# QuakeMigrate/QuakeMigrate

Measured on AMD Instinct MI355X. Metric: grid-nodes x time-samples stacked /sec (detect sweep), higher is better.
Workload: dtype f64

## Files before the change

quakemigrate_amd/csrc/qm_config.hip:

```cpp
#include "qm_config.hpp"

#include <cstring>

namespace {

using C = EngineConfig;

constexpr Tunable flag(const char *name, int C::*m, unsigned effects = 0) {
    return {name, m, nullptr, Tunable::kFlag, 0, 1, 0, {}, nullptr, effects};
}
constexpr Tunable range(const char *name, int C::*m, int64_t lo, int64_t hi, const char *refusal, unsigned effects = 0) {
    return {name, m, nullptr, Tunable::kRange, lo, hi, 0, {}, refusal, effects};
}
constexpr Tunable one_of(const char *name, int C::*m, int a, int b, int c, int d, const char *refusal,
                         unsigned effects = 0) {
    return {name, m, nullptr, Tunable::kSet, a, d, 4, {a, b, c, d}, refusal, effects};
}

}

const Tunable kTunables[] = {
    range("brick_x", &C::brick_x, 0, 64, "brick_x must be in 0..64 (0 = automatic)"),
    range("brick_y", &C::brick_y, 0, 64, "brick_y must be in 0..64 (0 = automatic)"),
    range("brick_z", &C::brick_z, 0, 64, "brick_z must be in 0..64 (0 = automatic)"),
    one_of("samples_per_lane", &C::samples_per_lane, 0, 1, 2, 4, "samples_per_lane must be 0 (automatic), 1, 2 or 4"),
    range("waves", &C::waves, 1, 16, "waves must be 1..16", kUserWaves),
    {"groups", &C::groups, nullptr, Tunable::kAtLeast, 0, 0, 0, {}, "groups must be >= 0", 0},
    range("rounds", &C::rounds, 1, 1024, "rounds must be in 1..1024", kUserRounds),
    range("lds_bytes", &C::lds_bytes, 1024, 160 * 1024, "lds_bytes must be in 1 KiB..160 KiB", kUserLds),
    flag("force_direct", &C::force_direct),
    flag("generic", &C::generic),
    flag("exact", &C::exact),
    range("scan_waves", &C::scan_waves, 1, 4096, "scan_waves must be in 1..4096"),
    {"chunk_bytes", nullptr, &C::chunk_bytes, Tunable::kAtLeast, 1 << 20, 0, 0, {}, "chunk_bytes must be >= 1 MiB", 0},
    range("pair", &C::pair, 0, 2, "pair must be 0 (off), 1 (automatic) or 2 (any scan length)"),
    flag("screen", &C::screen),
    one_of("screen_pairs", &C::screen_pairs, 0, 1, 2, 4, "screen_pairs must be 0, 1, 2 or 4", kVoidScreen),
    flag("screen_brick16", &C::screen_brick16, kVoidScreen),
    range("screen_big", &C::screen_big, -1, 1, "screen_big must be -1 (automatic), 0 or 1", kVoidScreen),
    range("shift", &C::shift, -1, 1, "shift must be -1 (automatic), 0 (off) or 1"),
    one_of("shift_waves", &C::shift_waves, 0, 4, 8, 12, "shift_waves must be 0 (automatic), 4, 8 or 12", kVoidShift),
    range("shift_lazy", &C::shift_lazy, -1, 1, "shift_lazy must be -1 (automatic), 0 or 1"),
    flag("shift_tail", &C::shift_tail),
    range("shift_rows_direct", &C::shift_rows_direct, 0, 2, "shift_rows_direct must be 0, 1 or 2", kVoidShift),
    range("shift_wide", &C::shift_wide, -1, 1, "shift_wide must be -1 (automatic), 0 (off) or 1"),
    range("shift_wide_rows", &C::shift_wide_rows, 0, 2,
          "shift_wide_rows must be 0 (never), 1 (where all rows do not fit) or 2 (always)", kVoidShiftWide),
    range("stream_pull", &C::stream_pull, -1, 1, "stream_pull must be -1 (slots of <= 1 MB), 0 (never) or 1 (always)"),
    flag("stream_stamps", &C::stream_stamps),
    flag("preproc_skew", &C::preproc_skew),
    range("tie_rule", &C::tie_rule, 0, 1, "tie_rule must be 0 (largest sum) or 1 (the reference's exp rule)"),
    flag("tie_sets", &C::tie_sets),
    flag("trigger_timing", &C::trigger_timing),
    flag("log_timing", &C::log_timing, kResetTimingLog),
};
const int kNumTunables = (int)(sizeof(kTunables) / sizeof(kTunables[0]));

static const Tunable *find_tunable(const char *key) {
    for (const Tunable &t : kTunables)
        if (std::strcmp(t.name, key) == 0) return &t;
    return nullptr;
}

int config_set(EngineConfig &c, const char *key, int64_t v, unsigned *effects) {
    const Tunable *t = find_tunable(key);
    if (!t) return fail("unknown config key '%s'", key);
    bool ok = true;
    switch (t->check) {
    case Tunable::kFlag: v = v ? 1 : 0; break;
    case Tunable::kRange: ok = v >= t->lo && v <= t->hi; break;
    case Tunable::kAtLeast: ok = v >= t->lo; break;
    case Tunable::kSet:
        ok = false;
        for (int i = 0; i < t->n_allowed; ++i) ok = ok || v == t->allowed[i];
        break;
    }
    if (!ok) return fail("%s", t->refusal);
    if (t->wide) c.*t->wide = v;
    else c.*t->member = (int)v;
    if (t->member == &C::lds_bytes) c.lds_bytes = (int)(v / 16 * 16);
    if ((t->member == &C::brick_x || t->member == &C::brick_y || t->member == &C::brick_z) && c.brick_x > 0) {
        if (c.brick_y < 1) c.brick_y = 1;
        if (c.brick_z < 1) c.brick_z = 1;
    }
    if (t->effects & kUserWaves) c.user_waves = true;
    if (t->effects & kUserRounds) c.user_rounds = true;
    if (t->effects & kUserLds) c.user_lds = true;
    if (effects) *effects = t->effects;
    return 0;
}

bool config_get(const EngineConfig &c, const char *key, int64_t *v) {
    const Tunable *t = find_tunable(key);
    if (!t) return false;
    *v = t->wide ? c.*t->wide : (int64_t)(c.*t->member);
    return true;
}
```

quakemigrate_amd/csrc/qm_config.hpp:

```cpp
#pragma once
#include <cstdint>

#pragma GCC visibility push(hidden)

int fail(const char *fmt, ...) __attribute__((format(printf, 1, 2)));

struct EngineConfig {
    int brick_x = 0, brick_y = 0, brick_z = 0;
    int samples_per_lane = 0;
    int waves = 8;
    bool user_waves = false, user_lds = false;
    int groups = 0;
    int rounds = 12;
    bool user_rounds = false;
    int lds_bytes = 80 * 1024;
    int force_direct = 0;
    int generic = 0;
    int scan_waves = 32;
    int exact = 1;
    int64_t chunk_bytes = (int64_t)4 << 30;
    int pair = 1;
    int screen = 0;
    int screen_pairs = 0;
    int screen_brick16 = 0;
    int screen_big = -1;
    int shift = -1;
    int shift_waves = 0;
    int shift_lazy = -1;
    int shift_tail = 1;
    int shift_rows_direct = 1;
    int shift_wide = -1;
    int shift_wide_rows = 1;
    int stream_pull = -1;
    int stream_stamps = 0;
    int preproc_skew = 1;
    int tie_rule = 0;
    int tie_sets = 1;
    int trigger_timing = 0;
    int log_timing = 0;
};

enum ConfigEffect : unsigned {
    kVoidShift = 1u << 0,
    kVoidShiftWide = 1u << 1,
    kVoidScreen = 1u << 2,
    kUserWaves = 1u << 3,
    kUserRounds = 1u << 4,
    kUserLds = 1u << 5,
    kResetTimingLog = 1u << 6,
};

struct Tunable {
    enum Check { kFlag, kRange, kAtLeast, kSet };
    const char *name;
    int EngineConfig::*member;
    int64_t EngineConfig::*wide;
    Check check;
    int64_t lo, hi;
    int n_allowed;
    int allowed[4];
    const char *refusal;
    unsigned effects;
};
extern const Tunable kTunables[];
extern const int kNumTunables;

int config_set(EngineConfig &c, const char *key, int64_t v, unsigned *effects);
bool config_get(const EngineConfig &c, const char *key, int64_t *v);

#pragma GCC visibility pop
```

quakemigrate_amd/csrc/qm_engine.hip:

```cpp
#define QM_TU_STEPS 1
#include "qm_engine.hpp"

namespace {

using qm::kPairLdsBytes;

qm::LaunchShape stack_shape(const qm_engine *e, const qm::StackArgs &a, int threads, size_t lds) {
    const int steps = a.n_steps > 1 ? a.n_steps : 1;
    return {(unsigned)(steps * a.ntiles * ((a.ngroups + 7) / 8 * 8)), threads, lds, e->stream};
}

bool pair_built(int S) { return S >= 1 && S <= qm::kPairMaxRows; }


bool shift_wanted(const qm_engine *e, int n_chunk, bool plain, bool volume, int64_t vol_stride) {
    if (!plain || e->cfg.shift == 0 || e->cfg.generic || e->cfg.force_direct ||
        e->cfg.user_waves || e->cfg.user_lds || e->cfg.samples_per_lane > 0 || e->cfg.pair == 2)
        return false;
    if (volume && vol_stride * 8 >= ((int64_t)1 << 32)) return false;
    if ((int64_t)e->g.ny * e->g.nz * 8 >= ((int64_t)1 << 32)) return false;
    return n_chunk >= 1;
}

int shift_tail_spl(const qm_engine *e, int rest) {
// ... 88 lines not shown
        p.cap_doubles = kPairLdsBytes / 8;
    }
    if (s.n_steps > 1) {
        p.batched = !volume && !marginal && !accumulate && s.run_if == nullptr && want_scan && (!shift || L->plain());
        if (!p.batched) {
            *out = p;
            return 0;
        }
        p.steps = s.n_steps;
    }
    if (!shift && jp == 0) {
        if (J != 1 && J != 2 && J != 4) return fail("samples_per_lane must be 1, 2 or 4 (got %d)", J);
        if (ensure_rel(e)) return 1;
    }
    if (marginal) p.marg_tiles = p.ntiles;
    const int n_wide_now = p.layout->n_list, nbricks_now = p.layout->g.nbricks;
    p.use_direct = e->cfg.force_direct || n_wide_now > 0;
    p.use_lds = !e->cfg.force_direct && n_wide_now < nbricks_now;
    p.direct_j = shift ? 4 : jp > 0 ? 2 * jp : J;
    p.direct_threads = shift ? 512 : jp > 0 ? 1024 : run_waves(e) * qm::kWave;
    p.direct_publish = (size_t)3 * (p.direct_threads / qm::kWave) * qm::kWave * p.direct_j * sizeof(double);
    const int threads = p.direct_threads;
    const int lds_blocks_per_cu =
        shift ? (L->nw == qm::kShiftWaves ? 2 : 1) : jp > 0 ? 1
               : std::max(1, std::min(160 * 1024 / std::max(1, run_lds_bytes(e)), 2048 / threads));
    if (p.use_lds) {
        int rounds = (!shift && jp == 0 && !e->cfg.user_rounds && e->g.brick_nodes <= 64) ? 3 : 0;
        if (shift && (wide || (L->nw == qm::kShiftWaves8 && L->nblk == 1)) && !e->cfg.user_rounds) {
            double best = 1e300;
            for (int r = 1; r <= e->cfg.rounds; ++r) {
                const int g = auto_groups(e, p.ntiles, nbricks_now, lds_blocks_per_cu, r);
                const double busy = (double)p.ntiles * g / ((double)r * e->n_cu * lds_blocks_per_cu);
                const double cost = (1.0 - std::min(1.0, busy)) + 0.002 * r;
                if (cost < best - 1e-9) { best = cost; rounds = r; }
            }
        }
        p.groups_lds = e->cfg.groups > 0 ? std::min(e->cfg.groups, nbricks_now)
                                         : auto_groups(e, p.ntiles, nbricks_now, lds_blocks_per_cu, rounds);
        p.brick_rows = (e->cfg.tie_rule && want_scan && e->cfg.tie_sets && shift && p.shift_mode == qm::kShiftDetect &&
                        L->plain()) ? nbricks_now : 0;
        if (e->cfg.tie_rule && want_scan && !p.brick_rows && !e->cfg.user_rounds && e->cfg.groups == 0) {
            const int fine = auto_groups(e, p.ntiles, std::max(1, nbricks_now / 4), lds_blocks_per_cu,
                                         8 * (rounds > 0 ? rounds : e->cfg.rounds));
            p.groups_lds = std::max(p.groups_lds, fine);
        }
        if (shift) {
            p.family = kFamilyShift;
            p.j = p.wide_tiles > 0 ? qm::kShiftWideSpl : 4;
            const bool per_brick = p.brick_rows && p.wide_tiles == 0;
            const int64_t life = (per_brick ? 1 : (int64_t)L->g.nbricks / std::max(1, p.groups_lds)) *
                                 std::max(1, L->g.brick_nodes / 8 / L->nw);
            p.lazy = e->cfg.shift_lazy >= 0 ? e->cfg.shift_lazy : (life >= qm::kShiftLazyGroups ? 1 : 0);
            if (L->nblk > 1 && !L->direct) p.lazy = 0;
        } else if (jp > 0) {
            p.family = kFamilyPair;
            p.j = 2 * jp;
        } else {
            const int S = e->g.n_rows;
            const bool exact = e->cfg.exact && !e->cfg.generic && !accumulate && qm::exact_built(S, J) &&
                               (marginal || !volume || S > qm::kPairMaxRows);
            p.family = exact ? kFamilyExact : kFamilyChunked;
            p.j = J;
        }
    }
    if (p.use_direct) {
        const int units = e->cfg.force_direct ? nbricks_now : n_wide_now;
        p.groups_direct = e->cfg.groups > 0 ? std::min(e->cfg.groups, units)
                                            : auto_groups(e, p.ntiles, units, 2048 / threads);
        p.list = e->cfg.force_direct ? nullptr : p.layout->list.p;
        p.n_list = units;
    }
    p.g = p.layout->g;
    p.sets = p.groups_lds + p.groups_direct;
    p.scan_n = p.steps * n_chunk;
    *out = p;
    return 0;
}

qm::StackArgs stack_args(const qm_engine *e, const StackLaunch &s, const StackPlan &p, bool direct) {
    const auto *vol = std::get_if<StackLaunch::Volume>(&s.kind);
    const auto *marg = std::get_if<StackLaunch::Marginal>(&s.kind);
    qm::StackArgs a{};
    a.g = p.g;
    a.onsets = s.onsets;
    a.lut = e->d_lut.p;
    if (!p.shift) {
        a.rel = p.layout->rel.p;
        a.brick_meta = p.layout->meta.p;
        a.brick_total = p.layout->total.p;
    }
    a.brick_list = direct ? p.list : nullptr;
    a.n_list = direct ? p.n_list : 0;
    a.T = s.T;
    a.fsmp = s.fsmp;
    a.n_samples = s.n_samples;
    a.sample0 = s.sample0;
    a.n_chunk = s.n_chunk;
    a.ntiles = direct && p.shift ? (s.n_chunk + qm::kShiftKT - 1) / qm::kShiftKT : p.ntiles;
    a.ngroups = direct ? p.groups_direct : p.groups_lds;
    a.tail_spl = direct ? 0 : p.tail_spl;
    a.wide_tiles = direct ? 0 : p.wide_tiles;
    if (p.steps > 1) {
        a.n_steps = p.steps;
        a.step_stride = s.step_stride;
    }
    a.part_stride = p.scan_n;
    a.cap_doubles = p.cap_doubles;
    a.z_scale = 1.4426950408889634074 / (double)s.available;
    a.volume = vol ? vol->p : nullptr;
    a.vol_stride = vol ? vol->stride : 0;
    a.accumulate = vol ? vol->accumulate : 0;
    a.part_max = e->d_pmax.p;
    a.part_idx = e->d_pidx.p;
    a.part_sum = e->d_psum.p;
    a.set0 = direct && p.use_lds ? p.groups_lds : 0;
    a.brick_max = p.brick_rows && !direct ? e->d_bmax.p : nullptr;
    a.want_scan = s.want_scan ? 1 : 0;
    a.marginal = marg ? e->d_marg.p : nullptr;
    a.m0 = marg ? marg->first : 0;
    a.m1 = marg ? marg->end : 0;
    a.n_nodes = e->n_nodes;
    a.run_if = s.run_if;
    return a;
}

int launch_round2_lds(qm_engine *e, const qm::StackArgs &a, StackPlan *p) {
    const int J = p->j, S = e->g.n_rows;
    const bool VOLUME = a.volume != nullptr || a.marginal != nullptr;
    const qm::LaunchShape shape = stack_shape(e, a, p->direct_threads,
                                              std::max((size_t)run_lds_bytes(e), p->direct_publish));
    bool exact = false;
    if (p->family == kFamilyExact) {
        const bool j4_wide = J == 4 && S > 40;
        if (a.marginal != nullptr) {
            if (S <= 32) QM_TABLE(qm::launch_exact_marginal_1_32(S, a, shape, &exact));
            else if (!j4_wide) QM_TABLE(qm::launch_exact_marginal_33_64(S, a, shape, &exact));
            else QM_TABLE(qm::launch_exact_marginal_j4_41_64(S, a, shape, &exact));
        } else if (!VOLUME) {
            if (S <= 32) QM_TABLE(qm::launch_exact_detect_1_32(S, a, shape, &exact));
            else if (!j4_wide) QM_TABLE(qm::launch_exact_detect_33_64(S, a, shape, &exact));
            else QM_TABLE(qm::launch_exact_detect_j4_41_64(S, a, shape, &exact));
        } else {
            if (!j4_wide) QM_TABLE(qm::launch_exact_volume_33_64(S, a, shape, &exact));
            else QM_TABLE(qm::launch_exact_volume_j4_41_64(S, a, shape, &exact));
        }
    }
    if (!exact) {
        p->family = kFamilyChunked;
        int nch = (e->cfg.generic || a.accumulate) ? 0 : e->g.row_pad / 8;
        if (nch > 8) nch = 0;
        bool built = false;
        if (VOLUME) QM_TABLE(qm::launch_chunked_volume(J, nch, a, shape, &built));
        else QM_TABLE(qm::launch_chunked_detect(J, nch, a, shape, &built));
        if (!built) return fail("no chunked stacking kernel for %d samples per lane", J);
    }
    return 0;
}

int launch_pair_lds(qm_engine *e, const qm::StackArgs &a) {
    bool done = false;
    const qm::LaunchShape shape = stack_shape(e, a, 1024, kPairLdsBytes);
    if (a.volume) QM_TABLE(qm::launch_pair_volume(e->g.n_rows, a, shape, &done));
    else QM_TABLE(qm::launch_pair_detect(e->g.n_rows, a, shape, &done));
    if (!done) return fail("no paired kernel built for %d rows", e->g.n_rows);
    return 0;
}

int launch_shift_lds(qm_engine *e, const qm::StackArgs &a, const StackPlan &p) {
    const ShiftLayout &L = *p.shift;
    const int mode = p.shift_mode;
    qm::ShiftArgs s{};
    s.a = a;
    s.smeta = reinterpret_cast<const int4 *>(L.meta.p);
    s.stotal = L.total.p;
    s.sfit = L.fit.p;
    s.stream = reinterpret_cast<const char *>(L.stream.p);
    s.wmeta = reinterpret_cast<const int4 *>(L.wmeta.p);
    s.wtotal = L.wtotal.p;
    s.wstream = reinterpret_cast<const char *>(L.wstream.p);
    s.rows2 = L.rows2;
    s.nw = L.nw;
    s.nblk = L.nblk;
    s.sb = L.sb;
    s.stage_slots = L.stage_slots;
    s.stage_reach = L.stage_reach;
    s.lazy = p.lazy;
    const qm::LaunchShape shape = stack_shape(e, a, L.nw * qm::kWave, qm::shift_lds_bytes(L.nw));
    const bool rows = L.nblk > 1, big = L.nw == qm::kShiftWaves8;
    if (L.wide && L.direct) QM_TABLE(qm::launch_shift_wide_rows(s, shape));
    else if (rows && L.quad && mode == qm::kShiftVolume) QM_TABLE(qm::launch_shift_rows4_volume(s, shape));
    else if (rows && L.quad) QM_TABLE(qm::launch_shift_rows4(s, shape));
    else if (rows && L.direct && mode == qm::kShiftVolume) QM_TABLE(qm::launch_shift_rows2_volume(s, shape));
    else if (rows && L.direct) QM_TABLE(qm::launch_shift_rows2(s, shape));
    else if (rows) QM_TABLE(qm::launch_shift_rows8(s, shape));
    else if (mode == qm::kShiftMarginal && big) QM_TABLE(qm::launch_shift_marginal8(s, shape));
    else if (mode == qm::kShiftMarginal) QM_TABLE(qm::launch_shift_marginal(s, shape));
    else if (mode == qm::kShiftVolume && big) QM_TABLE(qm::launch_shift_volume8(s, shape));
    else if (mode == qm::kShiftVolume) QM_TABLE(qm::launch_shift_volume(s, shape));
    else if (L.nw == qm::kShiftWaves3) QM_TABLE(qm::launch_shift_detect3(s, shape));
    else if (a.brick_max && big) QM_TABLE(qm::launch_shift_detect8_sets(s, shape));
    else if (a.brick_max) QM_TABLE(qm::launch_shift_detect_sets(s, shape));
    else if (big) QM_TABLE(qm::launch_shift_detect8(s, shape));
    else QM_TABLE(qm::launch_shift_detect(s, shape));
    return 0;
}

int launch_direct(qm_engine *e, const qm::StackArgs &a, const StackPlan &p) {
    const qm::LaunchShape shape = stack_shape(e, a, p.direct_threads, p.direct_publish);
    bool built = false;
    if (a.volume || a.marginal) QM_TABLE(qm::launch_direct_volume(p.direct_j, a, shape, &built));
    else QM_TABLE(qm::launch_direct_detect(p.direct_j, a, shape, &built));
    if (!built) return fail("no direct stacking kernel for %d samples per lane", p.direct_j);
    return 0;
}

int issue_stack(qm_engine *e, const StackLaunch &s, StackPlan *p) {
    if (p->marg_tiles && e->d_marg.ensure((size_t)p->marg_tiles * e->n_nodes)) return 1;
    const size_t rows_n = (size_t)p->brick_rows * p->scan_n;
    if (s.want_scan) {
        const size_t need = (size_t)p->sets * p->scan_n;
        if (e->d_pmax.ensure(need) || e->d_psum.ensure(need) || e->d_pidx.ensure(need)) return 1;
        if (p->brick_rows && e->d_bmax.ensure(rows_n)) return 1;
    }
    if (p->brick_rows && p->wide_tiles > 0) {
        hipLaunchKernelGGL(qm::fill_kernel, dim3((unsigned)std::min<size_t>((rows_n + 1023) / 1024, 65535)), dim3(256),
                           0, e->stream, e->d_bmax.p, rows_n, -std::numeric_limits<double>::infinity());
        QM_HIP(hipGetLastError());
    }
    const bool logged = s.run_if == nullptr;
    hipEvent_t ev_begin = nullptr, ev_end = nullptr;
    if (logged) {
        if (timing_events(e, &ev_begin, &ev_end)) return 1;
        QM_HIP(hipEventRecord(ev_begin, e->stream));
    }
    if (p->use_lds) {
        const qm::StackArgs a = stack_args(e, s, *p, false);
        if (p->family == kFamilyShift ? launch_shift_lds(e, a, *p)
            : p->family == kFamilyPair ? launch_pair_lds(e, a) : launch_round2_lds(e, a, p))
            return 1;
    }
    if (p->use_direct && launch_direct(e, stack_args(e, s, *p, true), *p)) return 1;
    if (logged) {
        QM_HIP(hipEventRecord(ev_end, e->stream));
        e->timed = !e->cfg.log_timing;
    }
    return 0;
}

}

int timing_events(qm_engine *e, hipEvent_t *begin, hipEvent_t *end) {
    *begin = e->ev0;
    *end = e->ev1;
    if (!e->cfg.log_timing) return 0;
    while (e->ev_used + 2 > e->ev_log.size()) {
        Event ev;
        QM_HIP(ev.create());
        e->ev_log.push_back(std::move(ev));
    }
    *begin = e->ev_log[e->ev_used];
    *end = e->ev_log[e->ev_used + 1];
    e->ev_used += 2;
    return 0;
}

StackResult run_stack(qm_engine *e, const StackLaunch &s) {
    e->last.sets_own = false;
    StackPlan p;
    if (plan_stack(e, s, &p)) return 1;
    StackResult r;
    r.batched = p.batched;
    if (!p.batched) return r;
    if (issue_stack(e, s, &p)) return 1;
    e->last = p;
    r.sets = p.sets;
    return r;
}

SetView engine_sets(const qm_engine *e, int n_sets, int n) {
// ... 172 lines not shown
}

int fetch_out(qm_engine *e, int n, int out_on_device, const OutSeries &st, const OutSeries &user) {
    if (out_on_device) return 0;
    void *dst[3] = {user.max, user.second, user.idx};
    QM_HIP(copy_back_pieces(dst, st.max, 3, (size_t)n * sizeof(double), e->stream));
    return 0;
}

namespace {

int finalize_sets(qm_engine *e, const SetView &in, int64_t n_nodes_total, const OutSeries &user, int out_on_device) {
    DeviceGuard guard(e->device);
    OutSeries st;
    if (stage_out(e, in.n, out_on_device, user, &st) || combine(e, in, kCombineFinal, 0, n_nodes_total, st, nullptr))
        return 1;
    return fetch_out(e, in.n, out_on_device, st, user);
}

struct Readout {
    const char *name;
    int64_t (*value)(const qm_engine *e);
    int (*fetch)(qm_engine *e);
};
int fetch_tie_counts(qm_engine *e) {
    if (!e->tie.counts_pending) return 0;
    int32_t h[2] = {0, 0};
    QM_HIP(copy_back(h, e->tie.count.p, sizeof(h), e->stream));
    e->tie.pairs_last = h[0];
    e->tie.overflow_last = h[1];
    e->tie.counts_pending = false;
    return 0;
}
#define V(expr) [](const qm_engine *e) -> int64_t { return (expr); }
const Readout kReadouts[] = {
    {"waves", V(run_waves(e))}, {"lds_bytes", V(run_lds_bytes(e))},
    {"screen_pairs", V(e->sweep.last_plan_jp)}, {"screen_big", V(e->sweep.last_plan_big)},
    {"shift_waves", V(e->last.shift && e->last.shift->ok ? e->last.shift->nw : e->sh.ok ? e->sh.nw : e->cfg.shift_waves)},
    {"screened_steps", V(e->sweep.screened_steps), drain_flags}, {"fallback_steps", V(e->sweep.fallback_steps), drain_flags},
    {"last_candidates", V(e->sweep.last_candidates), drain_flags}, {"screen_brick_nodes", V(e->screen.g.brick_nodes)},
    {"last_kernel", V(e->last.family)}, {"last_kernel_j", V(e->last.j)}, {"steps_per_launch", V(e->last_batched)},
    {"shift_tail_spl", V(e->last.tail_spl)}, {"shift_wide_tiles", V(e->last.wide_tiles)},
    {"shift_ok", V(e->sh.built && e->sh.ok ? 1 : 0)}, {"shift_wide_ok", V(e->shw.built && e->shw.ok ? 1 : 0)},
    {"shift_row_blocks", V(e->sh.ok ? e->sh.nblk : 0)}, {"shift_wide_row_blocks", V(e->shw.ok ? e->shw.nblk : 0)},
    {"shift_brick_nodes", V(e->sh.ok ? e->sh.g.brick_nodes : 0)},
    {"shift_wide_brick_nodes", V(e->shw.ok ? e->shw.g.brick_nodes : 0)},
    {"shift_wide_bricks", V(e->sh.ok ? e->sh.n_list : 0)}, {"shift_wide_direct_bricks", V(e->shw.ok ? e->shw.n_list : 0)},
    {"shift_operands_per_add_x1000",
     V(e->sh.ok && e->sh.group_rows > 0 ? (e->sh.quads * 4 * 1000) / (e->sh.group_rows * 32) : 0)},
    {"shift_wide_operands_per_add_x1000",
     V(e->shw.ok && e->shw.group_rows > 0 ? (e->shw.wquads * 4 * 1000) / (e->shw.group_rows * 48) : 0)},
    {"pair_brick_nodes", V(e->pair.kt ? e->pair.g.brick_nodes : 0)}, {"pair_tile", V(e->pair.ok ? e->pair.kt : 0)},
    {"pair_wide_bricks", V(e->pair.kt ? e->pair.n_list : 0)}, {"shift_lazy", V(e->last.lazy)},
    {"pick_lds_samples", V(qm::kPicksLdsSamples)}, {"amp_lds_samples", V(qm::kAmpLdsSamples)},
    {"trigger_max_radius", V(qm::kTrigMaxRadius)}, {"trigger_smooth_tile", V(qm::kTrigSmoothTile)},
    {"trigger_run_block", V(qm::kTrigRunBlock)}, {"trigger_merge_stride", V(qm::kTrigMergeThreads)},
    {"scanmseed_tile", V(qm::kSmsTile)}, {"scanmseed_compose_chunk", V(qm::kSmsComposeChunk)},
    {"tt_lds_nodes", V(qm::kTtLdsNodes)}, {"tt_section_threads", V(qm::kTtSectionThreads)},
    {"tt_grid_blocks", V(qm::kTtGridBlocks)}, {"tt_grid_threads", V(qm::kTtGridThreads)},
    {"tie_brick_rows", V(e->last.brick_rows)}, {"tie_refined_steps", V(e->tie.refined_steps)},
    {"tie_overflow_samples", V(e->tie.overflow_last), fetch_tie_counts}, {"tie_pairs", V(e->tie.pairs_last), fetch_tie_counts},
    {"table_hits", V(e->table_hits)}, {"table_misses", V(e->table_misses)}, {"table_evictions", V(e->table_evictions)},
    {"table_digests", V(e->table_digests)}, {"table_bytes", V(e->device_bytes())},
    {"tables_parked", V(std::count_if(e->slots.begin(), e->slots.end(), [](const TableSlot &sl) { return sl.used; }))},
    {"tables_parked_bytes", [](const qm_engine *e) -> int64_t {
         int64_t sum = 0;
         for (const TableSlot &sl : e->slots) sum += sl.used ? (int64_t)sl.state.device_bytes() : 0;
         return sum;
     }},
    {"pool_live_bytes", V(pool_live_bytes(e->device))},
    {"n_bricks", V(e->g.nbricks)},
    {"n_wide_bricks", V(e->r2().n_list), [](qm_engine *e) { return e->have_lut ? plan_wide(e, eff_j(e)) : 0; }},
    {"mean_span", [](const qm_engine *e) -> int64_t {
         int64_t sum = 0;
         const std::vector<int32_t> &totals = e->r2().h_total;
         for (int32_t t : totals) sum += t;
         return totals.empty() ? 0 : sum / ((int64_t)totals.size() * std::max(1, e->g.n_rows));
     }},
    {"n_cu", V(e->n_cu)}, {"n_nodes", V(e->n_nodes)}, {"n_rows", V(e->g.n_rows)},
    {"nx", V(e->g.nx)}, {"ny", V(e->g.ny)}, {"nz", V(e->g.nz)},
};
#undef V

template <int N>
bool clock_readout(const StageClock<N> &clock, const std::string &prefix, const std::string &key, int64_t *v) {
    for (int st = 0; st < N; ++st)
        if (key == prefix + clock.names[st]) return *v = clock.ns[st], true;
    return false;
}

}

extern "C" {

int qm_engine_create(int device_id, qm_engine **out) {
    if (!out) return fail("qm_engine_create: out is NULL");
    int n = 0;
    QM_HIP(hipGetDeviceCount(&n));
    if (device_id < 0 || device_id >= n)
        return fail("device %d not available (%d HIP devices visible)", device_id, n);
    DeviceGuard guard(device_id);
    std::unique_ptr<qm_engine, decltype(&qm_engine_destroy)> e(new qm_engine(), qm_engine_destroy);
    e->device = device_id;
    hipDeviceProp_t prop;
    QM_HIP(hipGetDeviceProperties(&prop, device_id));
    e->n_cu = prop.multiProcessorCount > 0 ? prop.multiProcessorCount : 256;
// ... 349 lines not shown
```

quakemigrate_amd/csrc/qm_engine.hpp:

```cpp
#pragma once
#include "../../include/qmhip.h"

#include <hip/hip_runtime.h>

#include <algorithm>
#include <atomic>
#include <cmath>
#include <cstdarg>
#include <cstdio>
#include <cstdlib>
#include <cstring>
#include <memory>
#include <mutex>
#include <string>
#include <thread>
#include <variant>
#include <vector>

#include "qm_config.hpp"
#include "qm_kernels.hpp"
#include "qm_launch.hpp"
#include "qm_screen.hpp"
#include "qm_pair.hpp"
#include "qm_shift.hpp"
// ... 310 lines not shown
    DevBuf<double> par;
    DevBuf<double> sec, out;
    DevBuf<double> tau;
    DevBuf<int32_t> meta;
    DevBuf<unsigned long long> bad;
    StageClock<qm::kTtStages> clock{qm::kTtStageNames};
};
struct TieScratch {
    DevBuf<double> zext, zgrid, z;
    DevBuf<int32_t> pairs, imin, count, cands;
    DevBuf<unsigned long long> emax, keys;
    int64_t refined_steps = 0, overflow_last = 0, pairs_last = 0;
    bool counts_pending = false;
};
struct ScreenScratch {
    DevBuf<int32_t> counts, cells, work, flags;
    DevBuf<int32_t> onq, cell, gmax, pm, sparams;
    DevBuf<double> rowmax, ssum, cand_z;
    DevBuf<int64_t> cand_idx;
    int64_t screened_steps = 0, fallback_steps = 0, last_candidates = 0;
    int last_plan_jp = 0, last_plan_big = 0;
    PinnedBuf<int32_t> h_flags;
    int flags_pending = 0, flags_head = 0;
};
struct FitScratch {
    DevBuf<double> a, b, c;
    DevBuf<double> part, val, win;
    DevBuf<int64_t> pidx;
};
struct CallStaging {
    DevBuf<double> sig;
    DevBuf<double> raw;
    DevBuf<double> pre_out;
    DevBuf<double> rs_raw;
};

struct StreamLane;

enum StackFamily : int { kFamilyChunked = 0, kFamilyExact = 1, kFamilyPair = 2, kFamilyShift = 3 };
struct StackPlan {
    StackFamily family = kFamilyChunked;
    int j = 0;
    const BrickLayout *layout = nullptr;
    const ShiftLayout *shift = nullptr;
    int shift_mode = 0, lazy = 0;
    int tail_spl = 0, wide_tiles = 0;
    int ntiles = 0, cap_doubles = 0;
    int steps = 1;
    bool use_lds = false, use_direct = false;
    int groups_lds = 0, groups_direct = 0;
    int direct_j = 0, direct_threads = 0;
    size_t direct_publish = 0;
    int brick_rows = 0;
    int marg_tiles = 0;
    bool batched = true;
    qm::GridDesc g{};
    const int32_t *list = nullptr;
    int n_list = 0;
    int sets = 0, scan_n = 0;
    bool sets_own = false;
};

struct qm_engine : TableState {
    int device = 0;
    std::vector<StreamLane *> streams;
    int n_cu = 256;
    hipStream_t own_stream = nullptr;
    hipStream_t stream = nullptr;
    Event ev0, ev1;
    bool timed = false;
    std::vector<Event> ev_log;
    size_t ev_used = 0;

    std::vector<TableSlot> slots;
    uint64_t cur_key = 0, table_clock = 0;
    bool cur_keyed = false;
    int64_t table_hits = 0, table_misses = 0, table_evictions = 0;
    int64_t table_digests = 0;
    DevBuf<unsigned long long> d_digest;

    EngineConfig cfg;

    DevBuf<int32_t> d_scalar;
    int last_batched = 1;
    StackPlan last;

    DevBuf<double> d_grids;
    DevBuf<int32_t> d_rows, d_served;
    int gx = 0, gy = 0, gz = 0, g_rows = 0;

    DevBuf<double> d_onsets, d_pmax, d_psum, d_bmax, d_out_a, d_chunk, d_marg, d_marg_out;
    DevBuf<int64_t> d_pidx;

    ResampleStage rs_stage;
    PreprocStage pre_stage;
    OnsetStage on_stage;
    CallStaging staging;
    PickStage picks;
    AmplitudeStage amps;
    TriggerStage trig;
    ScanmseedCodec sms;
    TravelTimeStage tt;
    TieScratch tie;
    ScreenScratch sweep;
    FitScratch fit;
};
// ... 188 lines not shown
```

quakemigrate_amd/csrc/qm_kernels.hpp:

```cpp
#pragma once

#include <hip/hip_runtime.h>
#include <stdint.h>

namespace qm {

constexpr int kWave = 64;
constexpr int64_t kNoIndex = INT64_MAX;
constexpr int kMaxSpanBytes = 65535;

struct GridDesc {
    int nx, ny, nz;
    int bx, by, bz;
    int nbx, nby, nbz;
    int nbricks;
    int brick_nodes;
    int n_rows;
    int row_pad;
};

struct StackArgs {
    GridDesc g;
    const double *onsets;
    const int32_t *lut;
    const uint16_t *rel;
    const int32_t *brick_meta;
    const int32_t *brick_total;
    const int32_t *brick_list;
    int n_list;
    int T, fsmp, n_samples;
    int sample0;
    int n_chunk;
    int ntiles, ngroups;
    int tail_spl;
    int wide_tiles;
    int n_steps;
    int64_t step_stride;
    int64_t part_stride;
    int cap_doubles;
    double z_scale;
    double *volume;
    int64_t vol_stride;
    int accumulate;
    double *part_max;
    int64_t *part_idx;
    double *part_sum;
    int set0;
    double *brick_max;
    int want_scan;
    double *marginal;
    int m0, m1;
    int64_t n_nodes;
    const int32_t *run_if;
};

__device__ __forceinline__ double max_keep(double best, double x) {
    double r;
    asm("v_max_f64 %0, %1, %2" : "=v"(r) : "v"(best), "v"(x));
    return r;
}

template <typename I>
__device__ __forceinline__ bool better(double v, I i, double best, I bi) {
    return (v > best) || (v == best && i < bi);
}

__device__ __forceinline__ void stack_tile_group(const StackArgs &a, int &tile, int &group) {
    const int slot = blockIdx.x >> 3;
    const int all = a.ntiles * (a.n_steps > 1 ? a.n_steps : 1);
    tile = (slot % all) % a.ntiles;
    group = (int)(blockIdx.x & 7) + 8 * (slot / all);
}
__device__ __forceinline__ StackArgs step_view(StackArgs a) {
    if (a.part_stride == 0) a.part_stride = a.n_chunk;
    if (a.n_steps > 1) {
        const int step = (int)((blockIdx.x >> 3) % (unsigned)(a.ntiles * a.n_steps)) / a.ntiles;
        a.onsets += (int64_t)step * a.step_stride;
        a.part_max += (int64_t)step * a.n_chunk;
        a.part_idx += (int64_t)step * a.n_chunk;
        a.part_sum += (int64_t)step * a.n_chunk;
        if (a.brick_max) a.brick_max += (int64_t)step * a.n_chunk;
    }
    return a;
}

__host__ __device__ __forceinline__ bool brick_fits(int64_t total_span, int n_rows, int kt,
                                                    int cap_doubles) {
    return total_span * 8 <= kMaxSpanBytes && total_span + (int64_t)n_rows * kt <= cap_doubles;
}

__device__ __forceinline__ void brick_extents(const GridDesc &g, int b, int &x0, int &y0, int &z0,
                                              int &vx, int &vy, int &vz) {
    const int bzi = b % g.nbz, byi = (b / g.nbz) % g.nby, bxi = b / (g.nbz * g.nby);
    x0 = bxi * g.bx; y0 = byi * g.by; z0 = bzi * g.bz;
    vx = min(g.bx, g.nx - x0); vy = min(g.by, g.ny - y0); vz = min(g.bz, g.nz - z0);
}

__device__ __forceinline__ int brick_walk_node(const GridDesc &g, int x0, int y0, int z0, int vy,
                                               int vz, int m) {
    const int lz = m % vz, ly = (m / vz) % vy, lx = m / (vz * vy);
    return ((x0 + lx) * g.ny + (y0 + ly)) * g.nz + (z0 + lz);
}

#ifdef QM_TU_TABLES
__global__ void brick_minmax_kernel(GridDesc g, const int32_t *__restrict__ lut,
                                    int4 *__restrict__ meta, int32_t *__restrict__ global_max) {
    const int b = blockIdx.x;
    int x0, y0, z0, vx, vy, vz;
    brick_extents(g, b, x0, y0, z0, vx, vy, vz);
    const int nvalid = vx * vy * vz;
    for (int r = threadIdx.x; r < g.n_rows; r += blockDim.x) {
        int lo = INT32_MAX, hi = 0;
        for (int m = 0; m < nvalid; ++m) {
            const int node = brick_walk_node(g, x0, y0, z0, vy, vz, m);
            int d = lut[(int64_t)node * g.n_rows + r];
            d = d < 0 ? 0 : d;
            lo = d < lo ? d : lo;
            hi = d > hi ? d : hi;
        }
        meta[(int64_t)b * g.n_rows + r] = make_int4(lo, hi - lo, 0, 0);
        atomicMax(global_max, hi);
    }
}
#endif

#ifdef QM_TU_TABLES
__global__ void brick_prefix_kernel(GridDesc g, int4 *__restrict__ meta,
                                    int32_t *__restrict__ btotal) {
    const int b = blockIdx.x * blockDim.x + threadIdx.x;
    if (b >= g.nbricks) return;
    int64_t run = 0;
    for (int r = 0; r < g.n_rows; ++r) {
        meta[(int64_t)b * g.n_rows + r].z = (int32_t)(run > INT32_MAX ? INT32_MAX : run);
        run += meta[(int64_t)b * g.n_rows + r].y;
// ... 1220 lines not shown
```

quakemigrate_amd/csrc/qm_shift.hpp:

```cpp
#pragma once

#include "qm_kernels.hpp"

namespace qm {

struct ShiftStageNext {
    const void *meta;
    int rows;
    int first_row, stride;
    const void *src;
    unsigned row_bytes;
    unsigned lds;
    unsigned lane32;
};

#ifndef QM_SHIFT_ASM_INC
#define QM_SHIFT_ASM_INC "qm_shift_asm.inc"
#endif
#include QM_SHIFT_ASM_INC

constexpr int kShiftWaves = 4;
constexpr int kShiftWaves8 = 8;
constexpr int kShiftWaves3 = 12;
constexpr int kShiftKT = 256;
// ... 329 lines not shown
                             "s_mov_b32 m0, %[ma]\n\t"
                             "s_nop 0\n\t"
                             "global_load_lds_dwordx4 %[vo], %[src]\n\t"
                             "s_mov_b64 exec, %[sv]"
                             : [sv] "=&s"(saved)
                             : [sh] "s"(__builtin_amdgcn_readfirstlane(kWave - pairs)),
                               [ma] "s"(__builtin_amdgcn_readfirstlane((int)(lds_base + 8u * (unsigned)(z4 + c)))),
                               [vo] "v"(lane16), [src] "s"(usrc + c)
                             : "memory", "m0");
            }
        } else {
            const int len = __builtin_amdgcn_readfirstlane(m.y) + kShiftWideKT;
            for (int u = lane; u < total; u += kWave) win[z4 + u] = (u < len && u < room) ? src[u] : 0.0;
        }
    }
    if ((S & 1) && wave == 0) {
        const int z4 = 4 * s.wtotal[vb];
        for (int u = lane; u < 4 * shift_zero_slots(1); u += kWave) win[z4 + u] = 0.0;
    }
}

struct ShiftWork {
    int tile, group, spl;
    int t_own;
    int t_first;
    bool run;
};
__device__ __forceinline__ ShiftWork shift_work(const StackArgs &a) {
    ShiftWork w;
    stack_tile_group(a, w.tile, w.group);
    w.run = w.group < a.ngroups && !(a.run_if != nullptr && *a.run_if == 0);
    if (w.tile < a.wide_tiles) {
        w.spl = kShiftWideSpl;
        w.t_own = w.tile * kShiftWideKT;
        w.t_first = w.t_own + kShiftWideKT > a.n_chunk ? a.n_chunk - kShiftWideKT : w.t_own;
        return w;
    }
    w.spl = (a.tail_spl > 0 && w.tile == a.ntiles - 1) ? a.tail_spl : 4;
    w.t_own = a.wide_tiles * kShiftWideKT + (w.tile - a.wide_tiles) * kShiftKT;
    w.t_first = (w.spl == 4 && w.t_own + kShiftKT > a.n_chunk && a.n_chunk >= kShiftKT)
                    ? a.n_chunk - kShiftKT : w.t_own;
    return w;
}
template <int J>
__device__ __forceinline__ void shift_reset(double (&vmax)[J], double (&vsum)[J], int (&vidx)[J]) {
#pragma unroll
    for (int k = 0; k < J; ++k) {
        vmax[k] = -__builtin_inf();
        vsum[k] = 0.0;
        vidx[k] = INT32_MAX;
    }
}

template <int NW, int J = 4>
__device__ __forceinline__ void shift_publish(const StackArgs &a, double *win, const double (&vmax)[J],
                                              const double (&vsum)[J], const int (&vidx)[J], int wave,
                                              int lane, int group, int t_first, int t_own = 0) {
    constexpr int KT = kWave * J;
    double *smax = win, *ssum = win + NW * KT;
    int *sidx = reinterpret_cast<int *>(win + 2 * NW * KT);
#pragma unroll
    for (int k = 0; k < J; ++k) {
        const int o = wave * KT + J * lane + k;
        smax[o] = vmax[k];
        ssum[o] = vsum[k];
        sidx[o] = vidx[k];
    }
    __syncthreads();
    const int k = threadIdx.x;
    if (k >= KT) return;
    double best = smax[k], total = ssum[k];
    int bi = sidx[k];
    for (int w = 1; w < NW; ++w) {
        const double v = smax[w * KT + k];
        const int i = sidx[w * KT + k];
        total += ssum[w * KT + k];
        if (better(v, i, best, bi)) {
            best = v;
            bi = i;
        }
    }
    const int t = t_first + k;
    if (t < a.n_chunk && t >= t_own) {
        const int64_t o = (int64_t)(a.set0 + group) * (a.part_stride ? a.part_stride : a.n_chunk) + t;
        a.part_max[o] = best;
        a.part_idx[o] = bi == INT32_MAX ? kNoIndex : (int64_t)bi;
        a.part_sum[o] = total;
    }
}

template <int MODE, int NW, int J, bool WIDE_LAZY = false, int SETS = 0>
__device__ __forceinline__ void shift_tile(const ShiftArgs &s, double *win, const ShiftWork &work,
                                           int lane, int wave) {
    constexpr bool kLdsState = NW == kShiftWaves3;
    constexpr bool kWide = J == kShiftWideSpl;
    constexpr bool kTail = J != 4;
    static_assert(!(kTail && kLdsState), "the 12-wave shape has no tail flavours");
    static_assert(!kWide || (MODE == kShiftDetect && NW == kShiftWaves8), "wide tiles: fused detect, 8 waves");
    static_assert(!SETS || (MODE == kShiftDetect && !kLdsState), "brick maxima: fused detect, 4 or 8 waves");
    static_assert(SETS != 2 || kWide, "brick maxima from the generated loop: wide tiles");
    const StackArgs &a = s.a;
    const GridDesc &g = a.g;
    const int tile = work.tile, group = work.group, t_first = work.t_first;
    const unsigned lds_base = (unsigned)(uintptr_t)((lds_f64 *)win);
    const unsigned lane_addr = lds_base + (unsigned)lane * (kTail ? 8u * J : 16u);
    const int seam = work.t_own - t_first;
// ... 20 lines not shown
    if constexpr (kLdsState) {
#pragma unroll
        for (int k = 0; k < 4; ++k) {
            state[(k / 2) * (kShiftStateChunk / 8) + (k & 1)] = vmax[k];
            state[(2 + k / 2) * (kShiftStateChunk / 8) + (k & 1)] = vsum[k];
            reinterpret_cast<int *>(state + 4 * (kShiftStateChunk / 8))[k] = vidx[k];
        }
    }
    (void)state_addr;
    constexpr int D = MODE == kShiftVolume ? Exp2Degree<true>::value
                      : MODE == kShiftMarginal ? kShiftMarginalDegree : Exp2Degree<false>::value;
    double c[D + 1];
#pragma unroll
    for (int i = 0; i <= D; ++i) c[i] = exp2_coeff<D>(i);

    const int64_t rpw = shift_recs_per_wave(g, s.rows2, NW);
    const int npairs = s.rows2 / 2, nz = g.nz, nynz = g.ny * g.nz;
    double *const marg_tile = a.marginal + (int64_t)tile * a.n_nodes;
    double *const vol_tile = a.volume + t_first;
    const unsigned vol_stride_bytes = (unsigned)(a.vol_stride * 8);
    (void)marg_tile; (void)vol_tile; (void)vol_stride_bytes;
    double wmax[J];
    int widx[J];
    (void)wmax; (void)widx;
    const int64_t brow_stride = a.part_stride ? a.part_stride : a.n_chunk;
    if constexpr (SETS == 1) {
#pragma unroll
        for (int k = 0; k < J; ++k) {
            wmax[k] = -__builtin_inf();
            widx[k] = INT32_MAX;
        }
    }
    auto brick_row = [&](int b) {
        constexpr int KT = kWave * J;
#pragma unroll
        for (int k = 0; k < J; ++k) win[wave * KT + J * lane + k] = vmax[k];
        __syncthreads();
        const int j = threadIdx.x;
        if (j < KT && t_first + j < a.n_chunk && t_first + j >= work.t_own) {
            double best = win[j];
            for (int w = 1; w < NW; ++w) best = win[w * KT + j] > best ? win[w * KT + j] : best;
            a.brick_max[(int64_t)b * brow_stride + t_first + j] = best;
        }
#pragma unroll
        for (int k = 0; k < J; ++k) {
            if (better(vmax[k], vidx[k], wmax[k], widx[k])) {
                wmax[k] = vmax[k];
                widx[k] = vidx[k];
            }
            vmax[k] = -__builtin_inf();
            vidx[k] = INT32_MAX;
        }
    };
    int prev = -1;
    for (int b = group; b < g.nbricks; b += a.ngroups) {
        if constexpr (SETS == 1) {
            if (prev >= 0) {
                __syncthreads();
                brick_row(prev);
            }
            prev = b;
        }
        if (!s.sfit[b]) continue;
#ifdef QM_SHIFT_EXP_NOSTAGE
        if (b == group) {
            if constexpr (kWide) {
                stage_shift_wide<NW>(s, win, b, g.n_rows, wave, lane, t_first);
                asm volatile("s_waitcnt vmcnt(0)" ::: "memory");
            } else {
                stage_shift_windows<NW>(s, win, b, 0, g.n_rows, g.n_rows, wave, lane, t_first);
            }
            __syncthreads();
        }
#else
        __syncthreads();
        if constexpr (kWide) {
            stage_shift_wide<NW>(s, win, b, g.n_rows, wave, lane, t_first);
            asm volatile("s_waitcnt vmcnt(0)" ::: "memory");
        } else {
            stage_shift_windows<NW, (NW == 12 ? 3 : 8), 6, kTail, kWave * J>(s, win, b, 0, g.n_rows, g.n_rows, wave,
                                                                             lane, t_first);
        }
        __syncthreads();
#endif
        int x0, y0, z0, vx, vy, vz, cx, cy, cz;
        shift_group_box(g, b, x0, y0, z0, vx, vy, vz, cx, cy, cz);
        const int nvg = cx * cy * cz;
        const int mine = (nvg - wave + NW - 1) / NW;
        if (mine <= 0) continue;
        const char *const stream = kWide ? s.wstream : s.stream;
        const char *run = stream + shift_run_record(b, wave, 0, NW, 1, rpw) * kShiftRec;
        int nb = b + a.ngroups;
        while (nb < g.nbricks && !s.sfit[nb]) nb += a.ngroups;
        const char *next_run = stream + shift_run_record(nb < g.nbricks ? nb : b, wave, 0, NW, 1, rpw) * kShiftRec;
        const unsigned next_off = (unsigned)lane * 64u;
        const void *next_meta = s.smeta + (int64_t)(nb < g.nbricks ? nb : b) * g.n_rows;
        (void)next_meta;
        const unsigned lane_addr_b = lane_addr + (unsigned)kShiftPlane8;
#ifdef QM_SHIFT_DEPHASE
        if (NW == kShiftWaves8 && (wave & 4)) __builtin_amdgcn_s_sleep(QM_SHIFT_DEPHASE);
#endif
        (void)lane_addr_b; (void)next_run; (void)next_off;
#define QM_TAIL_CALL(JJ)                                                                              \
        if constexpr (MODE == kShiftMarginal)                                                         \
            shift_tail##JJ##_marginal(vmax, vsum, vidx, run, mine, next_run, next_off, next_meta, npairs, lane_addr, nz, nynz,       \
                                      a.z_scale, c, marg_tile, weight, node_off, lane_x16, lane_x32); \
        else if constexpr (MODE == kShiftVolume)                                                      \
            shift_tail##JJ##_volume(vmax, vsum, vidx, run, mine, next_run, next_off, next_meta, npairs, lane_addr, nz, nynz,         \
                                    a.z_scale, c, vol_tile, vol_stride_bytes, (unsigned)lane * (8u * JJ), \
                                    slot_lanes);                                                      \
        else                                                                                          \
            shift_tail##JJ##_detect(vmax, vsum, vidx, run, mine, next_run, next_off, next_meta, npairs, lane_addr, nz, nynz,         \
                                    a.z_scale, c)
        const char *const brow = reinterpret_cast<const char *>(a.brick_max + (int64_t)b * brow_stride + t_first) -
                                 lds_base;
        (void)brow;
        if constexpr (kWide && WIDE_LAZY && SETS == 2)
            shift_wide_detect_bmax_lazy(vmax, vsum, vidx, run, mine, next_run, next_off, next_meta, npairs, lane_addr,
                                        brow, nz, nynz, a.z_scale, c);
        else if constexpr (kWide && SETS == 2)
            shift_wide_detect_bmax(vmax, vsum, vidx, run, mine, next_run, next_off, next_meta, npairs, lane_addr,
                                   brow, nz, nynz, a.z_scale, c);
        else if constexpr (kWide && WIDE_LAZY)
            shift_wide_detect_lazy(vmax, vsum, vidx, run, mine, next_run, next_off, next_meta, npairs, lane_addr, nz, nynz,
                                   a.z_scale, c);
        else if constexpr (kWide)
            shift_wide_detect(vmax, vsum, vidx, run, mine, next_run, next_off, next_meta, npairs, lane_addr, nz, nynz,
                              a.z_scale, c);
        else if constexpr (J == 1) { QM_TAIL_CALL(1); }
        else if constexpr (J == 2) { QM_TAIL_CALL(2); }
        else if constexpr (J == 3) { QM_TAIL_CALL(3); }
#undef QM_TAIL_CALL
        else if constexpr (kLdsState)
            shift_groups_detect3(run, mine, next_run, next_off, next_meta, npairs, lane_addr, state_addr, nz, nynz, a.z_scale, c);
        else if constexpr (NW == kShiftWaves8 && MODE == kShiftMarginal)
            shift_groups_marginal8(vmax, vsum, vidx, run, mine, next_run, next_off, next_meta, npairs, lane_addr, lane_addr_b, nz, nynz,
                                   a.z_scale, c, marg_tile, weight, node_off, lane_x16, lane_x32);
        else if constexpr (MODE == kShiftMarginal)
            shift_groups_marginal(vmax, vsum, vidx, run, mine, next_run, next_off, next_meta, npairs, lane_addr, nz, nynz, a.z_scale, c,
                                  marg_tile, weight, node_off, lane_x16, lane_x32);
        else if constexpr (NW == kShiftWaves8 && MODE == kShiftVolume)
            shift_groups_volume8(vmax, vsum, vidx, run, mine, next_run, next_off, next_meta, npairs, lane_addr, lane_addr_b, nz, nynz,
                                 a.z_scale, c, vol_tile, vol_stride_bytes, (unsigned)lane * 32u, store_lanes);
        else if constexpr (NW == kShiftWaves8) {
            if (s.lazy && SETS != 1)
                shift_groups_detect8_lazy(vmax, vsum, vidx, run, mine, next_run, next_off, next_meta, npairs, lane_addr, lane_addr_b, nz,
                                          nynz, a.z_scale, c);
            else
                shift_groups_detect8(vmax, vsum, vidx, run, mine, next_run, next_off, next_meta, npairs, lane_addr, lane_addr_b, nz, nynz,
                                     a.z_scale, c);
        }
        else if constexpr (MODE == kShiftVolume)
            shift_groups_volume(vmax, vsum, vidx, run, mine, next_run, next_off, next_meta, npairs, lane_addr, nz, nynz, a.z_scale, c,
                                vol_tile, vol_stride_bytes, (unsigned)lane * 32u, store_lanes);
        else if (s.lazy && SETS != 1)
            shift_groups_detect_lazy(vmax, vsum, vidx, run, mine, next_run, next_off, next_meta, npairs, lane_addr, nz, nynz, a.z_scale, c);
        else
            shift_groups_detect(vmax, vsum, vidx, run, mine, next_run, next_off, next_meta, npairs, lane_addr, nz, nynz, a.z_scale, c);
    }
    if (!a.want_scan) return;
    if constexpr (kLdsState) {
#pragma unroll
        for (int k = 0; k < 4; ++k) {
            vmax[k] = state[(k / 2) * (kShiftStateChunk / 8) + (k & 1)];
            vsum[k] = state[(2 + k / 2) * (kShiftStateChunk / 8) + (k & 1)];
            vidx[k] = reinterpret_cast<int *>(state + 4 * (kShiftStateChunk / 8))[k];
        }
    }
    __syncthreads();
    if constexpr (SETS == 1) {
        brick_row(prev);
#pragma unroll
        for (int k = 0; k < J; ++k) {
            vmax[k] = wmax[k];
            vidx[k] = widx[k];
        }
        __syncthreads();
    }
    shift_publish<NW, J>(a, win, vmax, vsum, vidx, wave, lane, group, t_first, work.t_own);
}

template <int MODE, int NW, bool SETS>
__device__ __forceinline__ void stack_shift_body(ShiftArgs &s, double *win) {
    static_assert(NW == kShiftWaves || NW == kShiftWaves8 || (NW == kShiftWaves3 && MODE == kShiftDetect),
                  "workgroup shapes: 4 or 8 waves, or 12 (detect only)");
    const int lane = threadIdx.x & (kWave - 1);
    const int wave = __builtin_amdgcn_readfirstlane(threadIdx.x >> 6);
    if constexpr (MODE == kShiftDetect) s.a = step_view(s.a);
    const ShiftWork work = shift_work(s.a);
    if (!work.run) return;
    if constexpr (MODE == kShiftDetect && NW == kShiftWaves8) {
        if (work.spl == kShiftWideSpl) {
            if constexpr (SETS) {
                if (s.lazy) return shift_tile<MODE, NW, kShiftWideSpl, true, 2>(s, win, work, lane, wave);
                return shift_tile<MODE, NW, kShiftWideSpl, false, 2>(s, win, work, lane, wave);
            }
            if (s.lazy) return shift_tile<MODE, NW, kShiftWideSpl, true, 0>(s, win, work, lane, wave);
            return shift_tile<MODE, NW, kShiftWideSpl, false, 0>(s, win, work, lane, wave);
        }
    }
    if constexpr (NW != kShiftWaves3) {
        if (work.spl == 3) return shift_tile<MODE, NW, 3, false, SETS ? 1 : 0>(s, win, work, lane, wave);
        if (work.spl == 2) return shift_tile<MODE, NW, 2, false, SETS ? 1 : 0>(s, win, work, lane, wave);
        if (work.spl == 1) return shift_tile<MODE, NW, 1, false, SETS ? 1 : 0>(s, win, work, lane, wave);
    }
    shift_tile<MODE, NW, 4, false, SETS ? 1 : 0>(s, win, work, lane, wave);
}

template <int MODE, int NW>
__global__ __launch_bounds__(NW * kWave, NW == kShiftWaves3 ? 3 : 2) void stack_shift_kernel(ShiftArgs s) {
    extern __shared__ __attribute__((aligned(16))) double win[];
    stack_shift_body<MODE, NW, false>(s, win);
// ... 451 lines not shown
```

Before: 584.6 billion.

## Seed lazy wide shift detect with a shared global running max per sample

Adds a global per-time-sample running-max buffer that workgroups in the lazy wide shift detect path fetch into LDS before each brick, fold into their register maxima, and publish back with atomic max. Seeding each group's maximum with the best value already found lets the lazy path skip more work, because candidates that cannot beat the global max are pruned earlier. In exchange it adds an extra fill, async LDS loads, inline-assembly atomics across groups, and ordering-dependent index handling that could affect tie behaviour.

Result: no change. 587.6 billion, median of 6 (+0.5%).

```diff
diff --git a/quakemigrate_amd/csrc/qm_config.hip b/quakemigrate_amd/csrc/qm_config.hip
--- a/quakemigrate_amd/csrc/qm_config.hip
+++ b/quakemigrate_amd/csrc/qm_config.hip
@@ -62,7 +62,14 @@
     return nullptr;
 }
 
+static bool is_shift_seed(const char *key) { return std::strcmp(key, "shift_seed") == 0; }
+
 int config_set(EngineConfig &c, const char *key, int64_t v, unsigned *effects) {
+    if (is_shift_seed(key)) {
+        c.shift_seed = v ? 1 : 0;
+        if (effects) *effects = 0;
+        return 0;
+    }
     const Tunable *t = find_tunable(key);
     if (!t) return fail("unknown config key '%s'", key);
     bool ok = true;
@@ -91,6 +98,7 @@
 }
 
 bool config_get(const EngineConfig &c, const char *key, int64_t *v) {
+    if (is_shift_seed(key)) return *v = c.shift_seed, true;
     const Tunable *t = find_tunable(key);
     if (!t) return false;
     *v = t->wide ? c.*t->wide : (int64_t)(c.*t->member);
diff --git a/quakemigrate_amd/csrc/qm_config.hpp b/quakemigrate_amd/csrc/qm_config.hpp
--- a/quakemigrate_amd/csrc/qm_config.hpp
+++ b/quakemigrate_amd/csrc/qm_config.hpp
@@ -27,6 +27,7 @@
     int shift = -1;
     int shift_waves = 0;
     int shift_lazy = -1;
+    int shift_seed = 1;
     int shift_tail = 1;
     int shift_rows_direct = 1;
     int shift_wide = -1;
diff --git a/quakemigrate_amd/csrc/qm_engine.hip b/quakemigrate_amd/csrc/qm_engine.hip
--- a/quakemigrate_amd/csrc/qm_engine.hip
+++ b/quakemigrate_amd/csrc/qm_engine.hip
@@ -164,6 +164,8 @@
                                  std::max(1, L->g.brick_nodes / 8 / L->nw);
             p.lazy = e->cfg.shift_lazy >= 0 ? e->cfg.shift_lazy : (life >= qm::kShiftLazyGroups ? 1 : 0);
             if (L->nblk > 1 && !L->direct) p.lazy = 0;
+            p.seeded = (e->cfg.shift_seed && p.lazy && p.wide_tiles > 0 && want_scan &&
+                        p.shift_mode == qm::kShiftDetect && L->plain() && !(e->cfg.tie_rule && !p.brick_rows)) ? 1 : 0;
         } else if (jp > 0) {
             p.family = kFamilyPair;
             p.j = 2 * jp;
@@ -227,6 +229,7 @@
     a.part_sum = e->d_psum.p;
     a.set0 = direct && p.use_lds ? p.groups_lds : 0;
     a.brick_max = p.brick_rows && !direct ? e->d_bmax.p : nullptr;
+    a.seed = p.seeded && !direct ? e->d_bmax.p + (size_t)p.brick_rows * p.scan_n : nullptr;
     a.want_scan = s.want_scan ? 1 : 0;
     a.marginal = marg ? e->d_marg.p : nullptr;
     a.m0 = marg ? marg->first : 0;
@@ -332,11 +335,13 @@
     if (s.want_scan) {
         const size_t need = (size_t)p->sets * p->scan_n;
         if (e->d_pmax.ensure(need) || e->d_psum.ensure(need) || e->d_pidx.ensure(need)) return 1;
-        if (p->brick_rows && e->d_bmax.ensure(rows_n)) return 1;
-    }
-    if (p->brick_rows && p->wide_tiles > 0) {
-        hipLaunchKernelGGL(qm::fill_kernel, dim3((unsigned)std::min<size_t>((rows_n + 1023) / 1024, 65535)), dim3(256),
-                           0, e->stream, e->d_bmax.p, rows_n, -std::numeric_limits<double>::infinity());
+        if ((p->brick_rows || p->seeded) && e->d_bmax.ensure(rows_n + (p->seeded ? p->scan_n : 0))) return 1;
+    }
+    if ((p->brick_rows && p->wide_tiles > 0) || p->seeded) {
+        const size_t first = p->brick_rows && p->wide_tiles > 0 ? 0 : rows_n;
+        const size_t fill_n = rows_n + (p->seeded ? p->scan_n : 0) - first;
+        hipLaunchKernelGGL(qm::fill_kernel, dim3((unsigned)std::min<size_t>((fill_n + 1023) / 1024, 65535)), dim3(256),
+                           0, e->stream, e->d_bmax.p + first, fill_n, -std::numeric_limits<double>::infinity());
         QM_HIP(hipGetLastError());
     }
     const bool logged = s.run_if == nullptr;
@@ -615,6 +620,7 @@
      V(e->shw.ok && e->shw.group_rows > 0 ? (e->shw.wquads * 4 * 1000) / (e->shw.group_rows * 48) : 0)},
     {"pair_brick_nodes", V(e->pair.kt ? e->pair.g.brick_nodes : 0)}, {"pair_tile", V(e->pair.ok ? e->pair.kt : 0)},
     {"pair_wide_bricks", V(e->pair.kt ? e->pair.n_list : 0)}, {"shift_lazy", V(e->last.lazy)},
+    {"shift_seeded", V(e->last.seeded)},
     {"pick_lds_samples", V(qm::kPicksLdsSamples)}, {"amp_lds_samples", V(qm::kAmpLdsSamples)},
     {"trigger_max_radius", V(qm::kTrigMaxRadius)}, {"trigger_smooth_tile", V(qm::kTrigSmoothTile)},
     {"trigger_run_block", V(qm::kTrigRunBlock)}, {"trigger_merge_stride", V(qm::kTrigMergeThreads)},
diff --git a/quakemigrate_amd/csrc/qm_engine.hpp b/quakemigrate_amd/csrc/qm_engine.hpp
--- a/quakemigrate_amd/csrc/qm_engine.hpp
+++ b/quakemigrate_amd/csrc/qm_engine.hpp
@@ -386,6 +386,7 @@
     int direct_j = 0, direct_threads = 0;
     size_t direct_publish = 0;
     int brick_rows = 0;
+    int seeded = 0;
     int marg_tiles = 0;
     bool batched = true;
     qm::GridDesc g{};
diff --git a/quakemigrate_amd/csrc/qm_kernels.hpp b/quakemigrate_amd/csrc/qm_kernels.hpp
--- a/quakemigrate_amd/csrc/qm_kernels.hpp
+++ b/quakemigrate_amd/csrc/qm_kernels.hpp
@@ -47,6 +47,7 @@
     double *part_sum;
     int set0;
     double *brick_max;
+    double *seed;
     int want_scan;
     double *marginal;
     int m0, m1;
@@ -80,6 +81,7 @@
         a.part_idx += (int64_t)step * a.n_chunk;
         a.part_sum += (int64_t)step * a.n_chunk;
         if (a.brick_max) a.brick_max += (int64_t)step * a.n_chunk;
+        if (a.seed) a.seed += (int64_t)step * a.n_chunk;
     }
     return a;
 }
diff --git a/quakemigrate_amd/csrc/qm_shift.hpp b/quakemigrate_amd/csrc/qm_shift.hpp
--- a/quakemigrate_amd/csrc/qm_shift.hpp
+++ b/quakemigrate_amd/csrc/qm_shift.hpp
@@ -405,6 +405,71 @@
     }
 }
 
+template <int J>
+__device__ __forceinline__ void shift_seed_look(const double *row, unsigned off, double (&seen)[J]) {
+    const double *p = reinterpret_cast<const double *>(reinterpret_cast<const char *>(row) + off);
+#pragma unroll
+    for (int k = 0; k < J; ++k) seen[k] = __hip_atomic_load(p + k, __ATOMIC_RELAXED, __HIP_MEMORY_SCOPE_AGENT);
+}
+__device__ __forceinline__ void shift_seed_fetch(const double *row, double *lds, int wave, int lane) {
+    static_assert(kShiftWideKT == 3 * 2 * kWave, "three wavefronts x 64 lanes x 16 bytes");
+    if (wave >= 3) return;
+    const unsigned long long sp = (unsigned long long)(row + 2 * kWave * wave);
+    const double *usrc = (const double *)(((unsigned long long)(unsigned)__builtin_amdgcn_readfirstlane((int)(sp >> 32)) << 32) |
+                                          (unsigned)__builtin_amdgcn_readfirstlane((int)sp));
+    const unsigned at = (unsigned)(uintptr_t)((lds_f64 *)lds) + 16u * kWave * (unsigned)wave;
+    asm volatile("s_mov_b32 m0, %[ma]\n\t"
+                 "s_nop 0\n\t"
+                 "global_load_lds_dwordx4 %[vo], %[src] sc1"
+                 :
+                 : [ma] "s"(__builtin_amdgcn_readfirstlane((int)at)), [vo] "v"((unsigned)lane * 16u), [src] "s"(usrc)
+                 : "memory", "m0");
+}
+__device__ __forceinline__ void shift_seed_exchange(double (&vmax)[6], int (&vidx)[6], const double *row,
+                                                    unsigned lane_addr, unsigned lds_base, unsigned lds_off, int go) {
+    unsigned long long saved;
+#define QM_SEED_SLOT(K, LO, HI, O)                                                                         \
+    "v_cmp_gt_f64 vcc, %[max" #K "], v[" #LO ":" #HI "]\n\t"                                            \
+    "s_and_saveexec_b64 %[sv], vcc\n\t"                                                                \
+    "global_atomic_max_f64 v60, %[max" #K "], %[row] offset:" #O "\n\t"                                  \
+    "s_mov_b64 exec, %[sv]\n\t"                                                                        \
+    "v_cmp_gt_f64 vcc, v[" #LO ":" #HI "], %[max" #K "]\n\t"                                            \
+    "v_cndmask_b32 %[idx" #K "], %[idx" #K "], v61, vcc\n\t"                                              \
+    "v_max_f64 %[max" #K "], %[max" #K "], v[" #LO ":" #HI "]\n\t"
+    asm volatile("s_cmp_eq_u32 %[go], 0\n\t"
+                 "s_cbranch_scc1 Lseed_done%=\n\t"
+                 "v_add_u32 v60, %[ldsoff], %[lane]\n\t"
+                 "ds_read_b64 v[48:49], v60\n\t"
+                 "ds_read_b64 v[50:51], v60 offset:8\n\t"
+                 "ds_read_b64 v[52:53], v60 offset:16\n\t"
+                 "ds_read_b64 v[54:55], v60 offset:24\n\t"
+                 "ds_read_b64 v[56:57], v60 offset:32\n\t"
+                 "ds_read_b64 v[58:59], v60 offset:40\n\t"
+                 "v_subrev_u32 v60, %[base], %[lane]\n\t"
+                 "v_mov_b32 v61, 0x7fffffff\n\t"
+                 "s_waitcnt lgkmcnt(0)\n\t"
+                 QM_SEED_SLOT(0, 48, 49, 0) QM_SEED_SLOT(1, 50, 51, 8) QM_SEED_SLOT(2, 52, 53, 16)
+                 QM_SEED_SLOT(3, 54, 55, 24) QM_SEED_SLOT(4, 56, 57, 32) QM_SEED_SLOT(5, 58, 59, 40)
+                 "Lseed_done%=:"
+                 : [max0] "+v"(vmax[0]), [max1] "+v"(vmax[1]), [max2] "+v"(vmax[2]), [max3] "+v"(vmax[3]),
+                   [max4] "+v"(vmax[4]), [max5] "+v"(vmax[5]), [idx0] "+v"(vidx[0]), [idx1] "+v"(vidx[1]),
+                   [idx2] "+v"(vidx[2]), [idx3] "+v"(vidx[3]), [idx4] "+v"(vidx[4]), [idx5] "+v"(vidx[5]),
+                   [sv] "=&s"(saved)
+                 : [go] "s"(go), [ldsoff] "s"(lds_off), [lane] "v"(lane_addr), [base] "s"(lds_base), [row] "s"(row)
+                 : "v48", "v49", "v50", "v51", "v52", "v53", "v54", "v55", "v56", "v57", "v58", "v59", "v60", "v61",
+                   "vcc", "scc", "memory");
+#undef QM_SEED_SLOT
+}
+template <int J>
+__device__ __forceinline__ void shift_seed_raise(double *row, unsigned off, const double (&seen)[J],
+                                                 const double (&vmax)[J]) {
+    double *p = reinterpret_cast<double *>(reinterpret_cast<char *>(row) + off);
+#pragma unroll
+    for (int k = 0; k < J; ++k)
+        if (vmax[k] > seen[k])
+            (void)__hip_atomic_fetch_max(p + k, vmax[k], __ATOMIC_RELAXED, __HIP_MEMORY_SCOPE_AGENT);
+}
+
 template <int NW, int J = 4>
 __device__ __forceinline__ void shift_publish(const StackArgs &a, double *win, const double (&vmax)[J],
                                               const double (&vsum)[J], const int (&vidx)[J], int wave,
@@ -531,6 +596,10 @@
             vidx[k] = INT32_MAX;
         }
     };
+    constexpr bool kSeed = kWide && WIDE_LAZY && SETS != 1;
+    const bool seeded = kSeed && a.seed != nullptr;
+    double *const seed_row = a.seed + t_first;
+    (void)seeded; (void)seed_row;
     int prev = -1;
     for (int b = group; b < g.nbricks; b += a.ngroups) {
         if constexpr (SETS == 1) {
@@ -541,7 +610,15 @@
             prev = b;
         }
         if (!s.sfit[b]) continue;
+        int seed_used = 0;
+        bool look = false;
+        if constexpr (kSeed) {
+            seed_used = 4 * (s.wtotal[b] + ((g.n_rows & 1) ? shift_zero_slots(1) : 0));
+            look = seeded && (seed_used + kShiftWideKT) * 8 <= kShiftLdsBytes8;
+        }
+        (void)seed_used; (void)look;
 #ifdef QM_SHIFT_EXP_NOSTAGE
+        look = false;
         if (b == group) {
             if constexpr (kWide) {
                 stage_shift_wide<NW>(s, win, b, g.n_rows, wave, lane, t_first);
@@ -554,6 +631,9 @@
 #else
         __syncthreads();
         if constexpr (kWide) {
+            if constexpr (kSeed) {
+                if (look) shift_seed_fetch(seed_row, win + seed_used, wave, lane);
+            }
             stage_shift_wide<NW>(s, win, b, g.n_rows, wave, lane, t_first);
             asm volatile("s_waitcnt vmcnt(0)" ::: "memory");
         } else {
@@ -567,6 +647,11 @@
         const int nvg = cx * cy * cz;
         const int mine = (nvg - wave + NW - 1) / NW;
         if (mine <= 0) continue;
+        if constexpr (kSeed) {
+            shift_seed_exchange(vmax, vidx, seed_row, lane_addr, lds_base,
+                                (unsigned)__builtin_amdgcn_readfirstlane(8 * seed_used),
+                                __builtin_amdgcn_readfirstlane(look ? 1 : 0));
+        }
         const char *const stream = kWide ? s.wstream : s.stream;
         const char *run = stream + shift_run_record(b, wave, 0, NW, 1, rpw) * kShiftRec;
         int nb = b + a.ngroups;
@@ -637,6 +722,14 @@
         else
             shift_groups_detect(vmax, vsum, vidx, run, mine, next_run, next_off, next_meta, npairs, lane_addr, nz, nynz, a.z_scale, c);
     }
+    if constexpr (kSeed) {
+        if (seeded) {
+            double seen[J];
+            const unsigned seed_off = lane_addr - lds_base;
+            shift_seed_look<J>(seed_row, seed_off, seen);
+            shift_seed_raise<J>(seed_row, seed_off, seen, vmax);
+        }
+    }
     if (!a.want_scan) return;
     if constexpr (kLdsState) {
 #pragma unroll
```
